# msg7086/x265-Yuuki-Asuna

Hardware: AMD Instinct MI355X
Metric: encoded fps + bit-exact check, 4K preset=slow, 1/2/4/8 MI355X vs host AVX2 (higher is better)
Workload: dtype u8; 1 GPU; 3840x2160 8-bit closed-loop frame pipeline (tier T2): lookahead -> exhaustive +-57 ME, 85 PUs/CTU -> subme 3 -> MC + DCT/quant/recon qp 27 -> deblock -> SAO (rdo) -> border -> next reference; parallelism=none (1 GPU), ctus_per_frame=2040

## Files before the change

x265-yuuki-asuna_amd/csrc/me_kernels.hip:

```cpp
#include "common.h"
#include <mutex>

#include <cstdlib>
#include <type_traits>

namespace x265hip {

struct MEArgs
{
    const uint8_t* fenc;  long fencStrideB;
    const uint8_t* fref;  long frefStrideB;
    int ctusW;
    int range;
    int rowBytes;
    int payloadDw;
    int32_t*  surf;
    unsigned long long* best;
    const uint16_t* costX;
    const uint16_t* costY;
    const int16_t* centres;
    int xcdOrder;
};

__device__ __forceinline__ void zorder_xy(int lane, int& bx, int& by)
// ... 581 lines not shown
                    }
                    else { if (p + 2 < 8) ldpair32(nxt, bb, p + 2); else ldpair32(nxt, bn, 0); }
                }
                u64 w0, w1;
                if (LD64 || LDA) { w0 = buf[(p >> 1) & 1][p & 1][0]; w1 = buf[(p >> 1) & 1][p & 1][1]; }
                else if (RING)
                {
                    const uint32_t (&dd)[3] = d3[(p >> 1) & 1][p & 1];
                    w0 = ((u64)dd[1] << 32) | dd[0]; w1 = ((u64)dd[2] << 32) | dd[1];
                }
                else { w0 = ((u64)cur[p & 1][1] << 32) | cur[p & 1][0]; w1 = ((u64)cur[p & 1][2] << 32) | cur[p & 1][1]; }
#pragma unroll
                for (int j = 0; j < 8; j++)
                {
                    if (FIRST && j > p) continue;
                    u64 v = j == 0 ? 0ull : acc[(p - j) & 7];
                    v = __builtin_amdgcn_qsad_pk_u16_u8(w0, F[j][0], v);
                    v = __builtin_amdgcn_qsad_pk_u16_u8(w1, F[j][1], v);
                    acc[(p - j) & 7] = v;
                }
                if (!FIRST || p == 7)
                {
                    const int m = mb + p;
                    const int slot = (p + 1) & 7;
                    const u64 A = acc[slot];
                    const uint32_t lo = (uint32_t)A, hi = (uint32_t)(A >> 32);
                    const uint32_t qlo = (uint32_t)quad_sum((int)lo), qhi = (uint32_t)quad_sum((int)hi);
                    uint32_t s80, s82;
                    if (MASK)
                    {
                        asm("v_and_b32 %0, 0xffff, %1" : "=v"(s80) : "v"(lo));
                        asm("v_and_b32 %0, 0xffff, %1" : "=v"(s82) : "v"(hi));
                    }
                    else { s80 = lo & 0xffffu; s82 = hi & 0xffffu; }
                    const uint32_t s81 = lo >> 16, s83 = hi >> 16;
                    const uint32_t v16 = __builtin_amdgcn_perm(qhi, qlo, selK);
                    const uint32_t v32 = (uint32_t)row_sum_of_quads((int)v16);
                    const uint32_t sb = CTAB ? (uint32_t)__builtin_amdgcn_readlane((int)cb, p) : (((uint32_t)a.costY[m] << 8) | (uint32_t)m);
                    if (COLMIN)
                    {
                        const uint32_t k0 = (s80 << 8) + sb, k1 = (s81 << 8) + sb, k2 = (s82 << 8) + sb, k3 = (s83 << 8) + sb;
                        r8c[0] = k0 < r8c[0] ? k0 : r8c[0];
                        r8c[1] = k1 < r8c[1] ? k1 : r8c[1];
                        r8c[2] = k2 < r8c[2] ? k2 : r8c[2];
                        r8c[3] = k3 < r8c[3] ? k3 : r8c[3];
                    }
                    else
                    {
                        const uint32_t k0 = (s80 << 2) + cxk4[0], k1 = (s81 << 2) + cxk4[1];
                        const uint32_t k2 = (s82 << 2) + cxk4[2], k3 = (s83 << 2) + cxk4[3];
                        uint32_t kmin = k0 < k1 ? k0 : k1;
                        kmin = k2 < kmin ? k2 : kmin;
                        kmin = k3 < kmin ? k3 : kmin;
                        uint32_t key = ((kmin & ~3u) << 8) + (sb << 2);
                        key = (key & ~3u) | (kmin & 3u);
                        r8 = key < r8 ? key : r8;
                    }
                    const uint32_t base = DEFERX ? sb : cxL8 + sb;
                    const uint32_t k16 = (v16 << 8) + base, k32 = (v32 << 8) + base;
                    r16 = k16 < r16 ? k16 : r16;
                    r32 = k32 < r32 ? k32 : r32;
                    if (!PAIR64 || FIRST)
                    {
                        v2u sw = __builtin_amdgcn_permlane16_swap(v32, v32, false, false);
                        const unsigned h64 = sw.x + sw.y;
                        sw = __builtin_amdgcn_permlane32_swap(h64, h64, false, false);
                        const uint32_t k64 = ((sw.x + sw.y) << 8) + base;
                        r64 = k64 < r64 ? k64 : r64;
                    }
                    else if ((p & 1) == 0) { v32even = v32; sbEven = sb; }
                    else if (QUAD64)
                    {
                        v2u sw = __builtin_amdgcn_permlane16_swap(v32even, v32, false, false);
                        const unsigned h64 = sw.x + sw.y;
                        const bool quadEnd = (p & 3) == 3, tailPair = (p & 3) == 1 && p + 2 >= NROWS;
                        if (quadEnd)
                        {
                            sw = __builtin_amdgcn_permlane32_swap(pairSum, h64, false, false);
                            uint32_t mine = pr[p >> 2];
                            if (!DEFERX) mine += cxL8;
                            const uint32_t k64 = ((sw.x + sw.y) << 8) + mine;
                            r64 = k64 < r64 ? k64 : r64;
                        }
                        else if (tailPair)
                        {
                            sw = __builtin_amdgcn_permlane32_swap(h64, h64, false, false);
                            uint32_t mine = pr[2 + (p >> 2)];
                            if (!DEFERX) mine += cxL8;
                            const uint32_t k64 = ((sw.x + sw.y) << 8) + mine;
                            r64 = k64 < r64 ? k64 : r64;
                        }
                        else pairSum = h64;
                    }
                    else
                    {
                        v2u sw = __builtin_amdgcn_permlane16_swap(v32even, v32, false, false);
                        const unsigned h64 = sw.x + sw.y;
                        sw = __builtin_amdgcn_permlane32_swap(h64, h64, false, false);
                        const uint32_t tot = sw.x + sw.y;
                        uint32_t mine = CTAB ? pr[p >> 1] : (oddRow ? sb : sbEven);
                        if (!DEFERX) mine += cxL8;
                        const uint32_t k64 = (tot << 8) + mine;
                        r64 = k64 < r64 ? k64 : r64;
                    }
                }
                if (!LD64 && !RING && !LDA && (p & 1))
                {
#pragma unroll
                    for (int q = 0; q < 2; q++) { cur[q][0] = nxt[q][0]; cur[q][1] = nxt[q][1]; cur[q][2] = nxt[q][2]; }
                }
                __builtin_amdgcn_sched_barrier(0);
            }
        };
        using I8 = std::integral_constant<int, 8>;
        rows8(std::true_type{}, I8{}, 0);
        int t0 = 8;
        for (; t0 + 8 <= T; t0 += 8)
            rows8(std::false_type{}, I8{}, t0);
        switch (T - t0)
        {
        case 2: rows8(std::false_type{}, std::integral_constant<int, 2>{}, t0); break;
        case 4: rows8(std::false_type{}, std::integral_constant<int, 4>{}, t0); break;
        case 6: rows8(std::false_type{}, std::integral_constant<int, 6>{}, t0); break;
        default: break;
        }
        {
            if (COLMIN)
            {
#pragma unroll
                for (int k = 0; k < 4; k++)
                {
                    const uint32_t kc = ((r8c[k] >> 8) << 2) + cxk4[k];
                    const uint32_t key = ((kc & ~3u) << 8) | ((r8c[k] & 255u) << 2) | (kc & 3u);
                    r8 = key < r8 ? key : r8;
                }
            }
            const u64 w8 = ((u64)(r8 >> 10) << 32) | (uint32_t)(((r8 >> 2) & 255u) * NC + 4 * g + (r8 & 3u));
            bk8 = w8 < bk8 ? w8 : bk8;
            auto widen = [&](const uint32_t r) { const uint32_t rc = DEFERX ? r + cxL8 : r; return ((u64)(rc >> 8) << 32) | (uint32_t)((rc & 255u) * NC + 4 * g + kcol); };
            const u64 w16 = widen(r16), w32 = widen(r32), w64 = widen(r64);
            bk16 = w16 < bk16 ? w16 : bk16;
            bk32 = w32 < bk32 ? w32 : bk32;
            bk64 = w64 < bk64 ? w64 : bk64;
        }
    }

    u64* rec = a.best + (size_t)ctu * 85;
    atomicMin(&rec[lane], bk8);
    atomicMin(&rec[64 + (lane >> 2)], bk16);
    if ((lane & 15) < 4) atomicMin(&rec[80 + (lane >> 4)], bk32);
    if ((lane & (QUAD64 ? 0x0f : PAIR64 ? 0x2f : 0x3f)) < 4) atomicMin(&rec[84], bk64);
}

template <bool SURF, bool BEST, int PITCH, int VAR = 1>
__global__ void __launch_bounds__(SURF && BEST ? 768 : 1024, SURF && BEST ? 3 : 4) me_ctu_w_kernel(MEArgs a)
{
    extern __shared__ __attribute__((aligned(16))) uint8_t win[];
    typedef unsigned long long u64;

    const int R = a.range;
    const int NC = 2 * R + 1;
    const int NG = (NC + 3) >> 2;
    const int rows = 64 + 2 * R;
    const int ctu = (gridDim.y == 1 && a.xcdOrder) ? xcd_swizzle((int)blockIdx.x, (int)gridDim.x) : (int)blockIdx.x;
    const int cx = (ctu % a.ctusW) * 64, cy = (ctu / a.ctusW) * 64;
    const int lane = threadIdx.x & 63;
    const int wave = __builtin_amdgcn_readfirstlane(threadIdx.x >> 6);
    const int nwaves = blockDim.x >> 6;
    constexpr int pitch = PITCH;

    const int ccx = a.centres ? a.centres[2 * ctu] : 0, ccy = a.centres ? a.centres[2 * ctu + 1] : 0;
    const uint8_t* g0 = a.fref + (long)(cy + ccy - R) * a.frefStrideB + (long)(cx + ccx - R) * 2;
    const int rowDw = a.payloadDw;
    for (int r = wave; r < rows; r += nwaves)
    {
        const uint8_t* src = g0 + (long)r * a.frefStrideB;
        uint32_t* dst = reinterpret_cast<uint32_t*>(win + lds_row_off(r, pitch));
        for (int c = lane; c < rowDw; c += 64)
            dst[c] = ld_u32(src + 4 * c);
    }
    int bx, by;
    zorder_xy(lane, bx, by);
    uint32_t F[8][4];
    {
        const uint8_t* fe = a.fenc + (long)(cy + by * 8) * a.fencStrideB + (long)(cx + bx * 8) * 2;
#pragma unroll
        for (int j = 0; j < 8; j++)
#pragma unroll
            for (int k = 0; k < 4; k++) F[j][k] = ld_u32(fe + (long)j * a.fencStrideB + 4 * k);
    }
    __syncthreads();

    u64 bk8 = ~0ull, bk16 = ~0ull, bk32 = ~0ull, bk64 = ~0ull;
    const int kcol = lane & 3;
    const bool is64 = lane >= 52 && lane < 56;
    const bool uMask = (lane & 15) < 4 || is64;
    const int uOffDw = is64 ? 84 * 4 + kcol : (80 + (lane >> 4)) * 4 + kcol;

    const int T = 2 * R + 8;
    for (int g = wave; g < NG; g += nwaves)
    {
        const uint8_t* colBase = win + (by * 8) * pitch + (bx * 8 + 4 * g) * 2;
        uint32_t cxk4[4] = { 0, 0, 0, 0 }, cxL = 0;
        uint32_t r8c[4] = { 0xffffffffu, 0xffffffffu, 0xffffffffu, 0xffffffffu };
        uint32_t r8 = 0xffffffffu, r16 = 0xffffffffu, r32 = 0xffffffffu, r64 = 0xffffffffu;
        if (BEST)
        {
#pragma unroll
            for (int k = 0; k < 4; k++)
                cxk4[k] = ((4 * g + k < NC ? (uint32_t)a.costX[4 * g + k] : (1u << 20)) << 2) | (uint32_t)k;
            cxL = 4 * g + kcol < NC ? (uint32_t)a.costX[4 * g + kcol] : (1u << 23);
        }
        const uint32_t cxL8 = cxL << 8;
        uint32_t acc[8][4];
#pragma unroll
        for (int i = 0; i < 8; i++)
#pragma unroll
            for (int k = 0; k < 4; k++) acc[i][k] = 0;

        auto row_step = [&](auto firstTag, const int t0, const int p)
        {
            constexpr bool FIRST = decltype(firstTag)::value;
            const int t = t0 + p;
            const uint32_t* lp = reinterpret_cast<const uint32_t*>(colBase + t * pitch + lds_skew_bytes(by + (t >> 3)));
            uint32_t d[6], e[5];
#pragma unroll
            for (int k = 0; k < 6; k++) d[k] = lp[k];
#pragma unroll
            for (int k = 0; k < 5; k++) e[k] = __builtin_amdgcn_alignbit(d[k + 1], d[k], 16);
#pragma unroll
            for (int j = 0; j < 8; j++)
            {
                if (FIRST && j > p) continue;
                const int slot = (p - j) & 7;
#pragma unroll
                for (int k = 0; k < 4; k++)
                {
                    acc[slot][0] = __builtin_amdgcn_sad_u16(d[k], F[j][k], acc[slot][0]);
                    acc[slot][1] = __builtin_amdgcn_sad_u16(e[k], F[j][k], acc[slot][1]);
                    acc[slot][2] = __builtin_amdgcn_sad_u16(d[k + 1], F[j][k], acc[slot][2]);
                    acc[slot][3] = __builtin_amdgcn_sad_u16(e[k + 1], F[j][k], acc[slot][3]);
                }
            }
            if (!FIRST || p == 7)
            {
                const int m = t - 7;
                const int slot = (p + 1) & 7;
                int s8[4], s16[4];
#pragma unroll
                for (int k = 0; k < 4; k++) { s8[k] = (int)acc[slot][k]; acc[slot][k] = 0; s16[k] = quad_sum(s8[k]); }
                const int v16 = kcol == 0 ? s16[0] : (kcol == 1 ? s16[1] : (kcol == 2 ? s16[2] : s16[3]));
                const int v32 = row_sum_of_quads(v16);
                typedef unsigned v2u __attribute__((ext_vector_type(2)));
                v2u sw = __builtin_amdgcn_permlane16_swap((unsigned)v32, (unsigned)v32, false, false);
                const unsigned h64 = sw.x + sw.y;
                sw = __builtin_amdgcn_permlane32_swap(h64, h64, false, false);
                const int v64 = (int)(sw.x + sw.y);
                if (SURF)
                {
                    typedef int v4i __attribute__((ext_vector_type(4)));
                    const u64 gofs = (u64)((((long)ctu * NC + m) * NG + g) * 340) * 4;
                    const u64 gsc = ((u64)__builtin_amdgcn_readfirstlane((uint32_t)(gofs >> 32)) << 32) | (uint32_t)__builtin_amdgcn_readfirstlane((uint32_t)gofs);
                    char* grp = reinterpret_cast<char*>(a.surf) + gsc;
                    const v4i v8 = { s8[0], s8[1], s8[2], s8[3] };
                    *reinterpret_cast<v4i*>(grp + (uint32_t)(lane * 16)) = v8;
                    *reinterpret_cast<int*>(grp + (uint32_t)(1024 + lane * 4)) = v16;
                    if (uMask) *reinterpret_cast<int*>(grp + (uint32_t)(uOffDw * 4)) = is64 ? v64 : v32;
                }
                if (BEST && !(VAR & 1))
                {
                    const uint32_t cy_ = a.costY[m];
                    {
                        const uint32_t k0 = ((uint32_t)s8[0] << 2) + cxk4[0], k1 = ((uint32_t)s8[1] << 2) + cxk4[1];
                        const uint32_t k2 = ((uint32_t)s8[2] << 2) + cxk4[2], k3 = ((uint32_t)s8[3] << 2) + cxk4[3];
                        uint32_t kmin = k0 < k1 ? k0 : k1;
                        kmin = k2 < kmin ? k2 : kmin;
                        kmin = k3 < kmin ? k3 : kmin;
                        const uint32_t rowc = (cy_ << 10) | ((uint32_t)m << 2);
                        uint32_t key = ((kmin & ~3u) << 8) + rowc;
                        key = (key & ~3u) | (kmin & 3u);
                        r8 = key < r8 ? key : r8;
                    }
                    const uint32_t cxy = cxL + cy_;
                    const uint32_t k16 = (((uint32_t)v16 + cxy) << 8) | (uint32_t)m;
                    const uint32_t k32 = (((uint32_t)v32 + cxy) << 8) | (uint32_t)m;
                    const uint32_t k64 = (((uint32_t)v64 + cxy) << 8) | (uint32_t)m;
                    r16 = k16 < r16 ? k16 : r16;
                    r32 = k32 < r32 ? k32 : r32;
                    r64 = k64 < r64 ? k64 : r64;
                }
                else if (BEST)
                {
                    const uint32_t rb = ((uint32_t)a.costY[m] << 8) | (uint32_t)m;
#pragma unroll
                    for (int k = 0; k < 4; k++)
                    {
                        const uint32_t kk = ((uint32_t)s8[k] << 8) + rb;
                        r8c[k] = kk < r8c[k] ? kk : r8c[k];
                    }
                    const uint32_t base = cxL8 + rb;
                    const uint32_t k16 = ((uint32_t)v16 << 8) + base;
                    const uint32_t k32 = ((uint32_t)v32 << 8) + base;
                    const uint32_t k64 = ((uint32_t)v64 << 8) + base;
                    r16 = k16 < r16 ? k16 : r16;
                    r32 = k32 < r32 ? k32 : r32;
                    r64 = k64 < r64 ? k64 : r64;
// ... 80 lines not shown
    }
    __syncthreads();

    u64 bk8 = ~0ull, bk16 = ~0ull, bk32 = ~0ull, bk64 = ~0ull;
    const int kcol = lane & 3;
    const int oddRow = (lane >> 4) & 1;
    const bool lane1 = (lane & 1) != 0, lane2 = (lane & 2) != 0;

    const int T = 2 * R + 8;
    const int gPer = groupsPerWg > 0 ? groupsPerWg : NG;
    const int gFirst = (int)blockIdx.y * gPer, gEnd = gFirst + gPer < NG ? gFirst + gPer : NG;
    for (int g = gFirst + wave; g < gEnd; g += nwaves)
    {
        const uint32_t colOff = (uint32_t)((by * 8) * pitch + (bx * 8 + 4 * g) * 2);
        auto block_off = [&](const int t0) { uint32_t o = colOff + (uint32_t)(t0 * pitch + lds_skew_bytes(by + (t0 >> 3))); asm volatile("" : "+v"(o)); return o; };
        uint32_t cxk4[4], cxL;
#pragma unroll
        for (int k = 0; k < 4; k++)
            cxk4[k] = ((4 * g + k < NC ? (uint32_t)a.costX[4 * g + k] : (1u << 20)) << 2) | (uint32_t)k;
        cxL = 4 * g + kcol < NC ? (uint32_t)a.costX[4 * g + kcol] : (1u << 23);
        const uint32_t cxL8 = cxL << 8;
        uint32_t r8c[4] = { 0xffffffffu, 0xffffffffu, 0xffffffffu, 0xffffffffu };
        uint32_t r8 = 0xffffffffu, r16 = 0xffffffffu, r32 = 0xffffffffu, r64 = 0xffffffffu;
        uint32_t acc[8][4];
#pragma unroll
        for (int i = 0; i < 8; i++)
#pragma unroll
            for (int k = 0; k < 4; k++) acc[i][k] = 0;

        auto tab = [&](const int i) { return ctab[i < 0 ? 0 : i]; };
        auto rows8 = [&](auto firstTag, auto nrowsTag, const int t0)
        {
            constexpr bool FIRST = decltype(firstTag)::value;
            constexpr int NROWS = decltype(nrowsTag)::value;
            const uint32_t bb = block_off(t0);
            const uint32_t cb = tab(t0 - 7 + (lane & 7));
            uint32_t v32even = 0, pairSum = 0, prq = 0;
#pragma unroll
            for (int p = 0; p < NROWS; p++)
            {
                if (!FIRST && (p & 3) == 0)
                    prq = tab(t0 - 7 + p + (p + 4 <= NROWS ? (lane >> 4) : oddRow));
                const uint32_t* lp = reinterpret_cast<const uint32_t*>(win + bb + p * pitch);
                uint32_t d[6], e[5];
#pragma unroll
                for (int k = 0; k < 6; k++) d[k] = lp[k];
#pragma unroll
                for (int k = 0; k < 5; k++) e[k] = __builtin_amdgcn_alignbit(d[k + 1], d[k], 16);
#pragma unroll
                for (int j = 0; j < 8; j++)
                {
                    if (FIRST && j > p) continue;
                    const int slot = (p - j) & 7;
#pragma unroll
                    for (int k = 0; k < 4; k++)
                    {
                        acc[slot][0] = __builtin_amdgcn_sad_u16(d[k], F[j][k], acc[slot][0]);
                        acc[slot][1] = __builtin_amdgcn_sad_u16(e[k], F[j][k], acc[slot][1]);
                        acc[slot][2] = __builtin_amdgcn_sad_u16(d[k + 1], F[j][k], acc[slot][2]);
                        acc[slot][3] = __builtin_amdgcn_sad_u16(e[k + 1], F[j][k], acc[slot][3]);
                    }
                }
                if (!FIRST || p == 7)
                {
                    const int slot = (p + 1) & 7;
                    int s8[4];
#pragma unroll
                    for (int k = 0; k < 4; k++) { s8[k] = (int)acc[slot][k]; acc[slot][k] = 0; }
                    const int keep0 = lane1 ? s8[1] : s8[0], give0 = lane1 ? s8[0] : s8[1];
                    const int keep1 = lane1 ? s8[3] : s8[2], give1 = lane1 ? s8[2] : s8[3];
                    const int t0s = keep0 + dpp<0xB1>(give0), t1s = keep1 + dpp<0xB1>(give1);
                    const int v16i = (lane2 ? t1s : t0s) + dpp<0x4E>(lane2 ? t0s : t1s);
                    const uint32_t v16 = (uint32_t)v16i;
                    const uint32_t v32 = (uint32_t)row_sum_of_quads(v16i);
                    const uint32_t sb = (uint32_t)__builtin_amdgcn_readlane((int)cb, p);
#pragma unroll
                    for (int k = 0; k < 4; k++)
                    {
                        const uint32_t kk = ((uint32_t)s8[k] << 8) + sb;
                        r8c[k] = kk < r8c[k] ? kk : r8c[k];
                    }
                    const uint32_t k16 = (v16 << 8) + sb, k32 = (v32 << 8) + sb;
                    r16 = k16 < r16 ? k16 : r16;
                    r32 = k32 < r32 ? k32 : r32;
                    if (FIRST)
                    {
                        v2u sw = __builtin_amdgcn_permlane16_swap(v32, v32, false, false);
                        const unsigned h64 = sw.x + sw.y;
                        sw = __builtin_amdgcn_permlane32_swap(h64, h64, false, false);
                        const uint32_t k64 = ((sw.x + sw.y) << 8) + sb;
                        r64 = k64 < r64 ? k64 : r64;
                    }
                    else if ((p & 1) == 0) v32even = v32;
                    else
                    {
                        v2u sw = __builtin_amdgcn_permlane16_swap(v32even, v32, false, false);
                        const unsigned h64 = sw.x + sw.y;
                        const bool quadEnd = (p & 3) == 3, tailPair = (p & 3) == 1 && p + 2 >= NROWS;
                        if (quadEnd)
                        {
                            sw = __builtin_amdgcn_permlane32_swap(pairSum, h64, false, false);
                            const uint32_t k64 = ((sw.x + sw.y) << 8) + prq;
                            r64 = k64 < r64 ? k64 : r64;
                        }
                        else if (tailPair)
                        {
                            sw = __builtin_amdgcn_permlane32_swap(h64, h64, false, false);
                            const uint32_t k64 = ((sw.x + sw.y) << 8) + prq;
                            r64 = k64 < r64 ? k64 : r64;
                        }
                        else pairSum = h64;
                    }
                }
                __builtin_amdgcn_sched_barrier(0);
            }
        };
        using I8 = std::integral_constant<int, 8>;
        rows8(std::true_type{}, I8{}, 0);
        int t0 = 8;
        for (; t0 + 8 <= T; t0 += 8)
            rows8(std::false_type{}, I8{}, t0);
        switch (T - t0)
        {
        case 2: rows8(std::false_type{}, std::integral_constant<int, 2>{}, t0); break;
        case 4: rows8(std::false_type{}, std::integral_constant<int, 4>{}, t0); break;
        case 6: rows8(std::false_type{}, std::integral_constant<int, 6>{}, t0); break;
        default: break;
        }
#pragma unroll
        for (int k = 0; k < 4; k++)
        {
            const uint32_t kc = ((r8c[k] >> 8) << 2) + cxk4[k];
            const uint32_t key = ((kc & ~3u) << 8) | ((r8c[k] & 255u) << 2) | (kc & 3u);
            r8 = key < r8 ? key : r8;
        }
        const u64 w8 = ((u64)(r8 >> 10) << 32) | (uint32_t)(((r8 >> 2) & 255u) * NC + 4 * g + (r8 & 3u));
        bk8 = w8 < bk8 ? w8 : bk8;
        auto widen = [&](const uint32_t r) { const uint32_t rc = r + cxL8; return ((u64)(rc >> 8) << 32) | (uint32_t)((rc & 255u) * NC + 4 * g + kcol); };
        const u64 w16 = widen(r16), w32 = widen(r32), w64 = widen(r64);
        bk16 = w16 < bk16 ? w16 : bk16;
        bk32 = w32 < bk32 ? w32 : bk32;
        bk64 = w64 < bk64 ? w64 : bk64;
    }
    u64* rec = a.best + (size_t)ctu * 85;
    atomicMin(&rec[lane], bk8);
    atomicMin(&rec[64 + (lane >> 2)], bk16);
    if ((lane & 15) < 4) { atomicMin(&rec[80 + (lane >> 4)], bk32); atomicMin(&rec[84], bk64); }
}

int launch_me_cand(const x265hip_me_params* p, hipStream_t s);

static const bool W2_DEFAULT = true;
static const int Q2_DEFAULT_FLAGS = 254;

struct MeEnv
{
    bool split, generic, cand;
    int bestVar;
    int q2Flags;
    int bestWaves;
    bool splitGroups8, splitGroups16;
    bool w2;
    bool xcdOrder;
};
static MeEnv g_meEnv;
static std::once_flag g_meEnvOnce;
static void me_env_read()
{
    MeEnv e;
    e.split = getenv("X265HIP_ME_SPLIT") != nullptr;
    e.generic = getenv("X265HIP_ME_GENERIC") != nullptr;
    const char* which = getenv("X265HIP_ME_KERNEL");
    e.cand = which && which[0] == 'c';
    const char* bv = getenv("X265HIP_ME_BEST_VARIANT");
    e.bestVar = bv ? atoi(bv) & 3 : -1;
    const char* q2 = getenv("X265HIP_ME_Q2_FLAGS");
    e.q2Flags = q2 ? atoi(q2) : (bv ? -1 : Q2_DEFAULT_FLAGS);
    e.xcdOrder = getenv("X265HIP_ME_XCD_OFF") == nullptr;
    e.bestWaves = getenv("X265HIP_ME_BEST_WAVES") ? atoi(getenv("X265HIP_ME_BEST_WAVES")) : 0;
    const char* sg = getenv("X265HIP_ME_SPLIT_GROUPS");
    e.splitGroups8 = !(sg && atoi(sg) == 0);
    e.splitGroups16 = sg && atoi(sg) == 1;
    const char* w2 = getenv("X265HIP_ME_W2");
    e.w2 = w2 ? atoi(w2) != 0 : W2_DEFAULT;
    g_meEnv = e;
}
static const MeEnv& me_env()
{
    std::call_once(g_meEnvOnce, me_env_read);
    return g_meEnv;
}
static int me_pitch_bytes(int bpp, int range)
{
    const int nld = bpp == 1 ? MECfg<uint8_t>::NLD : MECfg<uint16_t>::NLD;
    const int payload = (3 + (56 + 2 * range) * bpp + 4 * nld + 3) >> 2;
    const int payloadW = bpp == 2 ? (3 + (56 + 2 * range) * 2 + 4 * 6 + 3) >> 2 : payload;
    int pitchDw = 64;
    while (pitchDw < (payloadW > payload ? payloadW : payload) + 17) pitchDw <<= 1;
    return pitchDw * 4;
}

static int pick_waves(int ncols)
{
    return ncols >= 16 ? 16 : (ncols < 4 ? 4 : ncols);
}

template <typename Px>
static int launch_me(const x265hip_me_params* p, hipStream_t s)
{
    const MeEnv& env = me_env();
    const bool p_split = env.split;
    const bool p_generic = env.generic;
    constexpr int BPP = PxInfo<Px>::BPP;
    MEArgs a;
    a.fenc = (const uint8_t*)p->fenc;  a.fencStrideB = (long)p->fenc_stride * BPP;
    a.fref = (const uint8_t*)p->fref;  a.frefStrideB = (long)p->fref_stride * BPP;
    a.ctusW = p->width / 64;
    a.range = p->range;
    const int payload = (3 + (56 + 2 * p->range) * BPP + 4 * MECfg<Px>::NLD + 3) >> 2;
    a.payloadDw = payload;
    const int payloadW = sizeof(Px) == 2 ? (3 + (56 + 2 * p->range) * 2 + 4 * 6 + 3) >> 2 : payload;
    (void)payloadW;
    a.rowBytes = me_pitch_bytes(BPP, p->range);
    a.surf = p->surf; a.best = (unsigned long long*)p->best;
    const bool anySurf = p->surf != nullptr, anyBest = p->best != nullptr;
    const bool packed = anySurf && p->surf_format == X265HIP_SURF_PACKED;
    a.costX = p->cost_x; a.costY = p->cost_y;
    a.centres = p->centres;
    a.xcdOrder = env.xcdOrder ? 1 : 0;
    const int nctu = a.ctusW * (p->height / 64);
    const size_t lds = (size_t)a.rowBytes * (64 + 2 * p->range + 2);
    if (lds > 160 * 1024) { set_error("me_fullsearch: range %d needs %zu B of LDS (> 160 KiB)", p->range, lds); return X265HIP_EINVAL; }
    const int nw = pick_waves(2 * p->range + 1);
    dim3 grid(nctu), block(nw * 64);
#define LAUNCH_P(SF, BS, PT) do { \
        if (lds > 64 * 1024) X265HIP_TRY(hipFuncSetAttribute((const void*)me_ctu_kernel<Px, SF, BS, PT>, hipFuncAttributeMaxDynamicSharedMemorySize, (int)lds)); \
        hipLaunchKernelGGL((me_ctu_kernel<Px, SF, BS, PT>), grid, block, lds, s, a); } while (0)
#define LAUNCH(SF, BS) do { \
        if (a.rowBytes == 256) LAUNCH_P(SF, BS, 256); else if (a.rowBytes == 512) LAUNCH_P(SF, BS, 512); \
        else if (a.rowBytes == 1024) LAUNCH_P(SF, BS, 1024); \
        else { set_error("me_fullsearch: range %d needs an LDS row pitch of %d bytes (unsupported)", p->range, a.rowBytes); return X265HIP_EINVAL; } } while (0)
    {
        const bool wantT = p->surf && (p->surf_format == X265HIP_SURF_PACKED_T || p->surf_format == X265HIP_SURF_PACKED_B);
        if (sizeof(Px) == 1 && !p_generic && (wantT || env.cand))
        {
            const int rc = launch_me_cand(p, s);
            if (rc <= 0) return rc;
        }
        if (wantT)
        { set_error("me_fullsearch: X265HIP_SURF_PACKED_T / _PACKED_B are written by the record-per-lane kernel only (depth 8, window within its LDS / step limits)"); return X265HIP_EINVAL; }
    }
    if (sizeof(Px) == 1 && a.rowBytes == 256 && !p_generic)
    {
        const int bestVar = env.bestVar;
        const int q2Flags = env.q2Flags;
        const int bestWaves = env.bestWaves;
#define LAUNCH_QV(V) do { int nwq = pick_waves((2 * p->range + 4) / 4); if (nwq > 16) nwq = 16; if (nctu >= 1024 && nwq > 12) nwq = 12; \
        if (bestWaves >= 4 && bestWaves <= 16 && bestWaves < pick_waves((2 * p->range + 4) / 4) + 1) nwq = bestWaves; \
        hipLaunchKernelGGL((me_ctu_q_kernel<false, true, 256, false, V>), grid, dim3(nwq * 64), lds, s, a); } while (0)
#define LAUNCH_Q(SF, BS, MAXW) do { int nwq = pick_waves((2 * p->range + 4) / 4); if (nwq > (MAXW)) nwq = (MAXW); \
        if (packed) hipLaunchKernelGGL((me_ctu_q_kernel<SF, BS, 256, SF>), grid, dim3(nwq * 64), lds, s, a); \
        else hipLaunchKernelGGL((me_ctu_q_kernel<SF, BS, 256, false>), grid, dim3(nwq * 64), lds, s, a); } while (0)
        if (anySurf && anyBest && !p_split) LAUNCH_Q(true, true, 12);
        else
        {
            if (anySurf) LAUNCH_Q(true, false, 16);
            if (anyBest)
            {
                if (bestVar == 1) LAUNCH_QV(1); else if (bestVar == 2) LAUNCH_QV(2); else if (bestVar == 3) LAUNCH_QV(3);
                else if (q2Flags < 0) LAUNCH_QV(0);
                else
                {
                    int nwq = pick_waves((2 * p->range + 4) / 4); if (nwq > 16) nwq = 16; if (nctu >= 1024 && nwq > 8) nwq = 8;
                    if (bestWaves >= 4 && bestWaves <= 16 && bestWaves < pick_waves((2 * p->range + 4) / 4) + 1) nwq = bestWaves;
                    const bool splitGroups = env.splitGroups8;
                    const int ngroups = (2 * p->range + 4) / 4;
                    int gPer = 0;
                    dim3 grid2 = grid;
                    if (splitGroups && nctu < 192 && ngroups > 8) { nwq = 8; gPer = 8; grid2 = dim3(nctu, (ngroups + 7) / 8); }
                    const size_t ldsA = (size_t)320 * (64 + 2 * p->range + 2);
                    if ((q2Flags & 256) && (a.payloadDw + 24 > 80 || 2 * ldsA > 150 * 1024)) { set_error("me_fullsearch: X265HIP_ME_Q2_FLAGS bit 256 (two window copies) holds +-75 at most"); return X265HIP_EINVAL; }
                    const size_t ctabAt = (q2Flags & 256) ? 2 * ldsA : lds;
                    const size_t lds2 = ctabAt + (size_t)(2 * p->range + 1 + 16) * 4;
#define LAUNCH_Q2P(PT, FLV) case FLV: \
                        if (lds2 > 64 * 1024) X265HIP_TRY(hipFuncSetAttribute((const void*)me_ctu_q2_kernel<PT, FLV>, hipFuncAttributeMaxDynamicSharedMemorySize, (int)lds2)); \
                        hipLaunchKernelGGL((me_ctu_q2_kernel<PT, FLV>), grid2, dim3(nwq * 64), lds2, s, a, (int)ctabAt, gPer); break;
#define LAUNCH_Q2(FLV) LAUNCH_Q2P(256, FLV)
                    switch (q2Flags)
                    {
                    LAUNCH_Q2(0) LAUNCH_Q2(1) LAUNCH_Q2(2) LAUNCH_Q2(4) LAUNCH_Q2(8) LAUNCH_Q2(32) LAUNCH_Q2(62) LAUNCH_Q2(254) LAUNCH_Q2P(320, 446) LAUNCH_Q2P(320, 256)
                    default: set_error("me_fullsearch: X265HIP_ME_Q2_FLAGS %d is not an instantiated combination", q2Flags); return X265HIP_EINVAL;
                    }
#undef LAUNCH_Q2
#undef LAUNCH_Q2P
                }
            }
        }
#undef LAUNCH_Q
#undef LAUNCH_QV
    }
    else if (packed) { set_error("me_fullsearch: X265HIP_SURF_PACKED needs depth 8 and 2 * range + 75 <= 256"); return X265HIP_EINVAL; }
    else if (sizeof(Px) == 2 && p->depth <= 10 && (a.rowBytes == 512 || a.rowBytes == 256) && !p_generic)
    {
        const int plw = (3 + (56 + 2 * p->range) * 2 + 4 * 6 + 3) >> 2;
        a.payloadDw = plw > a.payloadDw ? plw : a.payloadDw;
        if (a.payloadDw + 17 > a.rowBytes / 4) { set_error("me_fullsearch: internal: window row does not fit the LDS pitch"); return X265HIP_EINVAL; }
        const int bestVarW = env.bestVar;
        const int bestWavesW = env.bestWaves;
#define LAUNCH_WV(V) do { int nwq = pick_waves((2 * p->range + 4) / 4); if (nwq > 16) nwq = 16; if (nctu >= 1024 && nwq > 12) nwq = 12;       \
        if (bestWavesW >= 4 && bestWavesW <= 16) nwq = bestWavesW; \
        if (a.rowBytes == 256) hipLaunchKernelGGL((me_ctu_w_kernel<false, true, 256, V>), grid, dim3(nwq * 64), lds, s, a); \
        else { \
            if (lds > 64 * 1024) X265HIP_TRY(hipFuncSetAttribute((const void*)me_ctu_w_kernel<false, true, 512, V>, hipFuncAttributeMaxDynamicSharedMemorySize, (int)lds)); \
            hipLaunchKernelGGL((me_ctu_w_kernel<false, true, 512, V>), grid, dim3(nwq * 64), lds, s, a); } } while (0)
#define LAUNCH_W(SF, BS, MAXW) do { int nwq = pick_waves((2 * p->range + 4) / 4); if (nwq > (MAXW)) nwq = (MAXW); \
        if (a.rowBytes == 256) hipLaunchKernelGGL((me_ctu_w_kernel<SF, BS, 256>), grid, dim3(nwq * 64), lds, s, a); \
        else { \
            if (lds > 64 * 1024) X265HIP_TRY(hipFuncSetAttribute((const void*)me_ctu_w_kernel<SF, BS, 512>, hipFuncAttributeMaxDynamicSharedMemorySize, (int)lds)); \
            hipLaunchKernelGGL((me_ctu_w_kernel<SF, BS, 512>), grid, dim3(nwq * 64), lds, s, a); } } while (0)
        if (anySurf && anyBest && !p_split) LAUNCH_W(true, true, 12);
        else
        {
            if (anySurf) LAUNCH_W(true, false, 16);
            if (anyBest)
            {
                const bool w2 = env.w2 && bestVarW < 0 && p->range <= 120;
                if (w2)
                {
                    int nwq = pick_waves((2 * p->range + 4) / 4); if (nwq > 16) nwq = 16; if (nctu >= 1024 && nwq > 12) nwq = 12;
                    if (bestWavesW >= 4 && bestWavesW <= 16) nwq = bestWavesW;
                    const bool splitGroupsW = env.splitGroups16;
                    const int ngroups = (2 * p->range + 4) / 4;
                    int gPer = 0;
                    dim3 grid2 = grid;
                    if (splitGroupsW && nctu < 192 && ngroups > 8) { nwq = 8; gPer = 8; grid2 = dim3(nctu, (ngroups + 7) / 8); }
                    const size_t lds2 = lds + (size_t)(2 * p->range + 1 + 16) * 4;
                    if (a.rowBytes == 256) hipLaunchKernelGGL((me_ctu_w2_kernel<256>), grid2, dim3(nwq * 64), lds2, s, a, (int)lds, gPer);
                    else
                    {
                        if (lds2 > 64 * 1024) X265HIP_TRY(hipFuncSetAttribute((const void*)me_ctu_w2_kernel<512>, hipFuncAttributeMaxDynamicSharedMemorySize, (int)lds2));
                        hipLaunchKernelGGL((me_ctu_w2_kernel<512>), grid2, dim3(nwq * 64), lds2, s, a, (int)lds, gPer);
                    }
                }
                else if (bestVarW == 0) LAUNCH_WV(0); else if (bestVarW == 2) LAUNCH_WV(2); else if (bestVarW == 3) LAUNCH_WV(3); else LAUNCH_WV(1);
            }
        }
#undef LAUNCH_W
#undef LAUNCH_WV
    }
    else if (anySurf && anyBest) LAUNCH(true, true);
    else if (anySurf) LAUNCH(true, false);
    else LAUNCH(false, true);
#undef LAUNCH
    X265HIP_TRY(hipGetLastError());
    return 0;
}

__global__ void fill_u64_kernel(unsigned long long* p, size_t n, unsigned long long v)
{
    size_t i = (size_t)blockIdx.x * blockDim.x + threadIdx.x;
    const size_t step = (size_t)gridDim.x * blockDim.x;
    for (; i < n; i += step) p[i] = v;
}

}

using namespace x265hip;

extern "C" const char* x265hip_me_minima_kernel_name(int depth, int range)
{
    static thread_local char name[64];
    const MeEnv& env = me_env();
    const int bpp = depth == 8 ? 1 : 2, pitch = me_pitch_bytes(bpp, range);
    if (depth != 8)
    {
        if (env.generic || depth > 10 || pitch > 512) return "me_ctu_kernel<u16,best>";
        return (env.w2 && env.bestVar < 0 && range <= 120) ? "me_ctu_w2_kernel" : "me_ctu_w_kernel<best>";
    }
    if (env.cand && !env.generic) return "me_ctu_c_kernel (record per lane)";
    if (env.generic || pitch != 256) return "me_ctu_kernel<u8,best>";
    if (env.q2Flags < 0 || range > 120 || env.bestVar > 0) return "me_ctu_q_kernel<best>";
    snprintf(name, sizeof(name), "me_ctu_q2_kernel<256,%d>", env.q2Flags);
    return name;
}

extern "C" void x265hip_me_env_refresh(void)
{
    (void)me_env();
    me_env_read();
}

extern "C" int x265hip_me_fullsearch(const x265hip_me_params* p, void* stream)
{
    int rc = ensure_device();
    if (rc) return rc;
    if (!p || !p->fenc || !p->fref) { set_error("me_fullsearch: NULL plane"); return X265HIP_EINVAL; }
    if (p->width <= 0 || p->height <= 0 || (p->width & 63) || (p->height & 63))
    { set_error("me_fullsearch: width/height must be positive multiples of 64 (got %dx%d)", p->width, p->height); return X265HIP_EINVAL; }
    if (p->range < 1 || p->range > 256) { set_error("me_fullsearch: range %d out of [1,256]", p->range); return X265HIP_EINVAL; }
    if (p->depth != 8 && p->depth != 10 && p->depth != 12) { set_error("me_fullsearch: depth %d", p->depth); return X265HIP_EINVAL; }
    const int bpp = p->depth == 8 ? 1 : 2;
    if (((p->fenc_stride * bpp) & 3) || ((p->fref_stride * bpp) & 3) || ((uintptr_t)p->fenc & 3))
    { set_error("me_fullsearch: plane strides must be multiples of 4 bytes and fenc 4-byte aligned"); return X265HIP_EINVAL; }
    const bool anyBest = p->best != nullptr;
    if (!p->surf && !p->best) { set_error("me_fullsearch: no output requested"); return X265HIP_EINVAL; }
    if (p->surf_format != X265HIP_SURF_I32 && p->surf_format != X265HIP_SURF_PACKED && p->surf_format != X265HIP_SURF_PACKED_T && p->surf_format != X265HIP_SURF_PACKED_B) { set_error("me_fullsearch: surf_format %d", p->surf_format); return X265HIP_EINVAL; }
    if (anyBest && (!p->cost_x || !p->cost_y)) { set_error("me_fullsearch: best[] needs cost_x / cost_y"); return X265HIP_EINVAL; }
    if (p->depth == 8) return launch_me<uint8_t>(p, (hipStream_t)stream);
    return launch_me<uint16_t>(p, (hipStream_t)stream);
}

extern "C" int x265hip_me_best_reset(uint64_t* best, size_t count, void* stream)
{
    int rc = ensure_device();
    if (rc) return rc;
    if (!best) { set_error("me_best_reset: NULL"); return X265HIP_EINVAL; }
    if (!count) return 0;
    int blocks = (int)((count + 255) / 256);
    if (blocks > 2048) blocks = 2048;
    hipLaunchKernelGGL(fill_u64_kernel, dim3(blocks), dim3(256), 0, (hipStream_t)stream,
                       (unsigned long long*)best, count, ~0ull);
    X265HIP_TRY(hipGetLastError());
    return 0;
}
```

Before: 625.4 frames/s.

## Add 8-column-group ME best-search kernel processing two column halves per wave

Adds me_ctu_o8_kernel, where each wave walks an 8-column group (two 4-column qsad halves) instead of 4 columns. Each LDS row load then feeds twice the SAD work, and the candidate cost-table fetches are amortised over both halves. It becomes the default 8-bit best-only path with 8 waves for large frames. In exchange it uses more accumulator registers per lane (acc[2][8]) and gets fewer waves per workgroup, which may lower occupancy or latency hiding.

```diff
diff --git a/x265-yuuki-asuna_amd/csrc/me_kernels.hip b/x265-yuuki-asuna_amd/csrc/me_kernels.hip
--- a/x265-yuuki-asuna_amd/csrc/me_kernels.hip
+++ b/x265-yuuki-asuna_amd/csrc/me_kernels.hip
@@ -757,6 +757,245 @@
     if ((lane & (QUAD64 ? 0x0f : PAIR64 ? 0x2f : 0x3f)) < 4) atomicMin(&rec[84], bk64);
 }
 
+template <int PITCH>
+__global__ void __launch_bounds__(1024, 4) me_ctu_o8_kernel(MEArgs a, int ctabOff, int groupsPerWg)
+{
+    extern __shared__ __attribute__((aligned(16))) uint8_t win[];
+    typedef unsigned long long u64;
+    typedef unsigned v2u __attribute__((ext_vector_type(2)));
+    const int R = a.range;
+    const int NC = 2 * R + 1;
+    const int NG = (NC + 7) >> 3;
+    const int rows = 64 + 2 * R;
+    const int ctu = (gridDim.y == 1 && a.xcdOrder) ? xcd_swizzle((int)blockIdx.x, (int)gridDim.x) : (int)blockIdx.x;
+    const int cx = (ctu % a.ctusW) * 64, cy = (ctu / a.ctusW) * 64;
+    const int lane = threadIdx.x & 63;
+    const int wave = __builtin_amdgcn_readfirstlane(threadIdx.x >> 6);
+    const int nwaves = blockDim.x >> 6;
+    constexpr int pitch = PITCH;
+
+    const int ccx = a.centres ? a.centres[2 * ctu] : 0, ccy = a.centres ? a.centres[2 * ctu + 1] : 0;
+    const uint8_t* g0 = a.fref + (long)(cy + ccy - R) * a.frefStrideB + (long)(cx + ccx - R);
+    const int rowDw = a.payloadDw;
+    for (int r = wave; r < rows; r += nwaves)
+    {
+        const uint8_t* src = g0 + (long)r * a.frefStrideB;
+        uint32_t* dst = reinterpret_cast<uint32_t*>(win + lds_row_off(r, pitch));
+        for (int c = lane; c < rowDw; c += 64)
+            dst[c] = ld_u32(src + 4 * c);
+    }
+    uint32_t* ctab = reinterpret_cast<uint32_t*>(win + ctabOff);
+    for (int i = threadIdx.x; i < NC + 16; i += blockDim.x)
+        ctab[i] = i < NC ? ((uint32_t)a.costY[i] << 8) | (uint32_t)i : 0xffffff00u;
+    uint32_t F[8][2];
+    {
+        int bx, by;
+        zorder_xy(lane, bx, by);
+        const uint8_t* fe = a.fenc + (long)(cy + by * 8) * a.fencStrideB + (long)(cx + bx * 8);
+#pragma unroll
+        for (int j = 0; j < 8; j++) { F[j][0] = ld_u32(fe + (long)j * a.fencStrideB); F[j][1] = ld_u32(fe + (long)j * a.fencStrideB + 4); }
+    }
+    __syncthreads();
+
+    u64* rec = a.best + (size_t)ctu * 85;
+    const uint32_t selK = 0x0c0c0000u | (uint32_t)((2 * (lane & 3) + 1) << 8) | (uint32_t)(2 * (lane & 3));
+
+    const int T = 2 * R + 8;
+    const int gPer = groupsPerWg > 0 ? groupsPerWg : NG;
+    const int gFirst = (int)blockIdx.y * gPer, gEnd = gFirst + gPer < NG ? gFirst + gPer : NG;
+    auto walk = [&](const int g, auto halvesTag)
+    {
+        constexpr int NH = decltype(halvesTag)::value;
+        int ln;
+        asm volatile("v_mbcnt_lo_u32_b32 %0, -1, 0\n\tv_mbcnt_hi_u32_b32 %0, -1, %0" : "=v"(ln));
+        int bx, by;
+        zorder_xy(ln, bx, by);
+        const int kcol = ln & 3;
+        const int oddRow = (ln >> 4) & 1;
+        const uint32_t colOff = (uint32_t)((by * 8) * pitch + bx * 8 + 8 * g);
+        auto block_off = [&](const int t0)
+        {
+            uint32_t o = colOff + (uint32_t)(t0 * pitch + lds_skew_bytes(by + (t0 >> 3)));
+            asm volatile("" : "+v"(o));
+            return o;
+        };
+        auto ldrow = [&](uint32_t (&d)[4], const uint32_t off, const int r)
+        {
+            const uint32_t* lp = reinterpret_cast<const uint32_t*>(win + off + r * pitch);
+            d[0] = lp[0]; d[1] = lp[1]; d[2] = lp[2]; d[3] = lp[3];
+        };
+        uint32_t r16[2] = { 0xffffffffu, 0xffffffffu }, r32[2] = { 0xffffffffu, 0xffffffffu }, r64[2] = { 0xffffffffu, 0xffffffffu };
+        uint32_t r8c[2][4];
+#pragma unroll
+        for (int h = 0; h < 2; h++)
+#pragma unroll
+            for (int k = 0; k < 4; k++) r8c[h][k] = 0xffffffffu;
+        u64 acc[2][8];
+#pragma unroll
+        for (int i = 0; i < 8; i++) { acc[0][i] = 0; acc[1][i] = 0; }
+        uint32_t d4[2][4];
+        ldrow(d4[0], block_off(0), 0);
+
+        uint32_t cbNext = 0;
+        auto fetch_consts = [&](const int t0)
+        {
+            int l;
+            asm volatile("v_mbcnt_lo_u32_b32 %0, -1, 0\n\tv_mbcnt_hi_u32_b32 %0, -1, %0" : "=v"(l));
+            const int i0 = t0 - 7 + (l & 7);
+            cbNext = ctab[i0 < 0 ? 0 : i0];
+        };
+        fetch_consts(0);
+
+        auto rows8 = [&](auto firstTag, auto nrowsTag, const int t0)
+        {
+            constexpr bool FIRST = decltype(firstTag)::value;
+            constexpr int NROWS = decltype(nrowsTag)::value;
+            const uint32_t bb = block_off(t0), bn = block_off(t0 + 8);
+            uint32_t bb4 = bb + 4 * pitch;
+            asm volatile("" : "+v"(bb4));
+            const uint32_t cb = cbNext;
+            uint32_t pr[4] = { 0, 0, 0, 0 };
+            if (!FIRST)
+            {
+                const int a0 = t0 - 7 + (lane >> 4);
+                if (NROWS >= 4) pr[0] = ctab[a0];
+                if (NROWS == 8) pr[1] = ctab[a0 + 4];
+                if (NROWS == 2 || NROWS == 6) pr[2 + (NROWS - 2) / 4] = ctab[t0 - 7 + (NROWS - 2) + oddRow];
+            }
+            fetch_consts(t0 + 8);
+            uint32_t v32even[2] = { 0, 0 }, pairSum[2] = { 0, 0 };
+#pragma unroll
+            for (int p = 0; p < NROWS; p++)
+            {
+                if (p + 1 < 4) ldrow(d4[(p + 1) & 1], bb, p + 1);
+                else if (p + 1 < 8) ldrow(d4[(p + 1) & 1], bb4, p + 1 - 4);
+                else ldrow(d4[(p + 1) & 1], bn, 0);
+                __builtin_amdgcn_sched_barrier(0);
+                const uint32_t (&dd)[4] = d4[p & 1];
+                const u64 w0 = ((u64)dd[1] << 32) | dd[0], w1 = ((u64)dd[2] << 32) | dd[1], w2 = ((u64)dd[3] << 32) | dd[2];
+#pragma unroll
+                for (int j = 0; j < 8; j++)
+                {
+                    if (FIRST && j > p) continue;
+                    const int s = (p - j) & 7;
+                    u64 va = j == 0 ? 0ull : acc[0][s];
+                    va = __builtin_amdgcn_qsad_pk_u16_u8(w0, F[j][0], va);
+                    va = __builtin_amdgcn_qsad_pk_u16_u8(w1, F[j][1], va);
+                    acc[0][s] = va;
+                    if (NH == 2)
+                    {
+                        u64 vb = j == 0 ? 0ull : acc[1][s];
+                        vb = __builtin_amdgcn_qsad_pk_u16_u8(w1, F[j][0], vb);
+                        vb = __builtin_amdgcn_qsad_pk_u16_u8(w2, F[j][1], vb);
+                        acc[1][s] = vb;
+                    }
+                }
+                if (!FIRST || p == 7)
+                {
+                    const int slot = (p + 1) & 7;
+                    const uint32_t sb = (uint32_t)__builtin_amdgcn_readlane((int)cb, p);
+#pragma unroll
+                    for (int h = 0; h < NH; h++)
+                    {
+                        const u64 A = acc[h][slot];
+                        const uint32_t lo = (uint32_t)A, hi = (uint32_t)(A >> 32);
+                        const uint32_t qlo = (uint32_t)quad_sum((int)lo), qhi = (uint32_t)quad_sum((int)hi);
+                        uint32_t s80, s82;
+                        asm("v_and_b32 %0, 0xffff, %1" : "=v"(s80) : "v"(lo));
+                        asm("v_and_b32 %0, 0xffff, %1" : "=v"(s82) : "v"(hi));
+                        const uint32_t s81 = lo >> 16, s83 = hi >> 16;
+                        const uint32_t v16 = __builtin_amdgcn_perm(qhi, qlo, selK);
+                        const uint32_t v32 = (uint32_t)row_sum_of_quads((int)v16);
+                        const uint32_t k0 = (s80 << 8) + sb, k1 = (s81 << 8) + sb, k2 = (s82 << 8) + sb, k3 = (s83 << 8) + sb;
+                        r8c[h][0] = k0 < r8c[h][0] ? k0 : r8c[h][0];
+                        r8c[h][1] = k1 < r8c[h][1] ? k1 : r8c[h][1];
+                        r8c[h][2] = k2 < r8c[h][2] ? k2 : r8c[h][2];
+                        r8c[h][3] = k3 < r8c[h][3] ? k3 : r8c[h][3];
+                        const uint32_t k16 = (v16 << 8) + sb, k32 = (v32 << 8) + sb;
+                        r16[h] = k16 < r16[h] ? k16 : r16[h];
+                        r32[h] = k32 < r32[h] ? k32 : r32[h];
+                        if (FIRST)
+                        {
+                            v2u sw = __builtin_amdgcn_permlane16_swap(v32, v32, false, false);
+                            const unsigned h64 = sw.x + sw.y;
+                            sw = __builtin_amdgcn_permlane32_swap(h64, h64, false, false);
+                            const uint32_t k64 = ((sw.x + sw.y) << 8) + sb;
+                            r64[h] = k64 < r64[h] ? k64 : r64[h];
+                        }
+                        else if ((p & 1) == 0) v32even[h] = v32;
+                        else
+                        {
+                            v2u sw = __builtin_amdgcn_permlane16_swap(v32even[h], v32, false, false);
+                            const unsigned h64 = sw.x + sw.y;
+                            const bool quadEnd = (p & 3) == 3, tailPair = (p & 3) == 1 && p + 2 >= NROWS;
+                            if (quadEnd)
+                            {
+                                sw = __builtin_amdgcn_permlane32_swap(pairSum[h], h64, false, false);
+                                const uint32_t k64 = ((sw.x + sw.y) << 8) + pr[p >> 2];
+                                r64[h] = k64 < r64[h] ? k64 : r64[h];
+                            }
+                            else if (tailPair)
+                            {
+                                sw = __builtin_amdgcn_permlane32_swap(h64, h64, false, false);
+                                const uint32_t k64 = ((sw.x + sw.y) << 8) + pr[2 + (p >> 2)];
+                                r64[h] = k64 < r64[h] ? k64 : r64[h];
+                            }
+                            else pairSum[h] = h64;
+                        }
+                    }
+                }
+                __builtin_amdgcn_sched_barrier(0);
+            }
+        };
+        using I8 = std::integral_constant<int, 8>;
+        rows8(std::true_type{}, I8{}, 0);
+        int t0 = 8;
+        for (; t0 + 8 <= T; t0 += 8)
+            rows8(std::false_type{}, I8{}, t0);
+        switch (T - t0)
+        {
+        case 2: rows8(std::false_type{}, std::integral_constant<int, 2>{}, t0); break;
+        case 4: rows8(std::false_type{}, std::integral_constant<int, 4>{}, t0); break;
+        case 6: rows8(std::false_type{}, std::integral_constant<int, 6>{}, t0); break;
+        default: break;
+        }
+        u64 bk8 = ~0ull, bk16 = ~0ull, bk32 = ~0ull, bk64 = ~0ull;
+#pragma unroll
+        for (int h = 0; h < NH; h++)
+        {
+            const uint32_t col0 = (uint32_t)(8 * g + 4 * h);
+            uint32_t cxk4[4];
+#pragma unroll
+            for (int k = 0; k < 4; k++)
+                cxk4[k] = (((int)col0 + k < NC ? (uint32_t)a.costX[col0 + k] : (1u << 20)) << 2) | (uint32_t)k;
+            const uint32_t cxL8 = ((int)col0 + kcol < NC ? (uint32_t)a.costX[col0 + kcol] : (1u << 23)) << 8;
+            uint32_t r8 = 0xffffffffu;
+#pragma unroll
+            for (int k = 0; k < 4; k++)
+            {
+                const uint32_t kc = ((r8c[h][k] >> 8) << 2) + cxk4[k];
+                const uint32_t key = ((kc & ~3u) << 8) | ((r8c[h][k] & 255u) << 2) | (kc & 3u);
+                r8 = key < r8 ? key : r8;
+            }
+            const u64 w8 = ((u64)(r8 >> 10) << 32) | (uint32_t)(((r8 >> 2) & 255u) * NC + col0 + (r8 & 3u));
+            bk8 = w8 < bk8 ? w8 : bk8;
+            auto widen = [&](const uint32_t r) { const uint32_t rc = r + cxL8; return ((u64)(rc >> 8) << 32) | (uint32_t)((rc & 255u) * NC + col0 + kcol); };
+            const u64 w16 = widen(r16[h]), w32 = widen(r32[h]), w64 = widen(r64[h]);
+            bk16 = w16 < bk16 ? w16 : bk16;
+            bk32 = w32 < bk32 ? w32 : bk32;
+            bk64 = w64 < bk64 ? w64 : bk64;
+        }
+        atomicMin(&rec[lane], bk8);
+        atomicMin(&rec[64 + (lane >> 2)], bk16);
+        if ((lane & 15) < 4) { atomicMin(&rec[80 + (lane >> 4)], bk32); atomicMin(&rec[84], bk64); }
+    };
+    for (int g = gFirst + wave; g < gEnd; g += nwaves)
+    {
+        if (8 * g + 4 >= NC) walk(g, std::integral_constant<int, 1>{});
+        else walk(g, std::integral_constant<int, 2>{});
+    }
+}
+
 template <bool SURF, bool BEST, int PITCH, int VAR = 1>
 __global__ void __launch_bounds__(SURF && BEST ? 768 : 1024, SURF && BEST ? 3 : 4) me_ctu_w_kernel(MEArgs a)
 {
@@ -1143,6 +1382,8 @@
 
 static const bool W2_DEFAULT = true;
 static const int Q2_DEFAULT_FLAGS = 254;
+static const bool O8_DEFAULT = true;
+static const int O8_WAVES_4K = 8;
 
 struct MeEnv
 {
@@ -1153,6 +1394,7 @@
     bool splitGroups8, splitGroups16;
     bool w2;
     bool xcdOrder;
+    bool o8;
 };
 static MeEnv g_meEnv;
 static std::once_flag g_meEnvOnce;
@@ -1174,6 +1416,8 @@
     e.splitGroups16 = sg && atoi(sg) == 1;
     const char* w2 = getenv("X265HIP_ME_W2");
     e.w2 = w2 ? atoi(w2) != 0 : W2_DEFAULT;
+    const char* o8 = getenv("X265HIP_ME_O8");
+    e.o8 = (o8 ? atoi(o8) != 0 : O8_DEFAULT) && !q2 && !bv && !which;
     g_meEnv = e;
 }
 static const MeEnv& me_env()
@@ -1189,6 +1433,12 @@
     int pitchDw = 64;
     while (pitchDw < (payloadW > payload ? payloadW : payload) + 17) pitchDw <<= 1;
     return pitchDw * 4;
+}
+
+static bool o8_serves(int payloadDw, int range)
+{
+    const int ng8 = (2 * range + 8) / 8;
+    return 4 * payloadDw >= 64 + 8 * ng8 && payloadDw + 17 <= 256 / 4;
 }
 
 static int pick_waves(int ncols)
@@ -1258,7 +1508,20 @@
             if (anySurf) LAUNCH_Q(true, false, 16);
             if (anyBest)
             {
-                if (bestVar == 1) LAUNCH_QV(1); else if (bestVar == 2) LAUNCH_QV(2); else if (bestVar == 3) LAUNCH_QV(3);
+                if (env.o8 && o8_serves(a.payloadDw, p->range))
+                {
+                    const int ngroups = (2 * p->range + 8) / 8;
+                    int nwq = ngroups < 4 ? 4 : (ngroups > 16 ? 16 : ngroups);
+                    if (nctu >= 1024) nwq = O8_WAVES_4K;
+                    if (bestWaves >= 4 && bestWaves <= 16) nwq = bestWaves;
+                    int gPer = 0;
+                    dim3 grid2 = grid;
+                    if (env.splitGroups8 && nctu < 192 && ngroups > 8) { nwq = 8; gPer = 8; grid2 = dim3(nctu, (ngroups + 7) / 8); }
+                    const size_t lds2 = lds + (size_t)(2 * p->range + 1 + 16) * 4;
+                    if (lds2 > 64 * 1024) X265HIP_TRY(hipFuncSetAttribute((const void*)me_ctu_o8_kernel<256>, hipFuncAttributeMaxDynamicSharedMemorySize, (int)lds2));
+                    hipLaunchKernelGGL((me_ctu_o8_kernel<256>), grid2, dim3(nwq * 64), lds2, s, a, (int)lds, gPer);
+                }
+                else if (bestVar == 1) LAUNCH_QV(1); else if (bestVar == 2) LAUNCH_QV(2); else if (bestVar == 3) LAUNCH_QV(3);
                 else if (q2Flags < 0) LAUNCH_QV(0);
                 else
                 {
@@ -1371,6 +1634,7 @@
     if (env.cand && !env.generic) return "me_ctu_c_kernel (record per lane)";
     if (env.generic || pitch != 256) return "me_ctu_kernel<u8,best>";
     if (env.q2Flags < 0 || range > 120 || env.bestVar > 0) return "me_ctu_q_kernel<best>";
+    if (env.o8 && o8_serves((3 + 56 + 2 * range + 4 * MECfg<uint8_t>::NLD + 3) >> 2, range)) return "me_ctu_o8_kernel<256>";
     snprintf(name, sizeof(name), "me_ctu_q2_kernel<256,%d>", env.q2Flags);
     return name;
 }
```

After: 625.2 frames/s, median of 3. About the same (-0.0%).
